# bcaitech1/p4-fr-sorry-math-but-love-you

Hardware: NVIDIA B200
Metric: EfficientSATRN greedy-decode images/sec (higher is better)
Workload: dtype bf16

## Files before the change

### p4-fr-sorry-math-but-love-you_b200/csrc/common.cuh

```cuda
#pragma once
#include <cuda_runtime.h>
#include <cuda_bf16.h>
#include <cuda_fp16.h>
#include <stdint.h>

#if defined(__CUDA_ARCH__) && (__CUDA_ARCH__ < 1000)
#error "frx is written for sm_100a (B200) only"
#endif

namespace frx {

enum Act : int { ACT_NONE = 0, ACT_RELU = 1, ACT_SILU = 2, ACT_SIGMOID = 3, ACT_GELU = 4 };

__device__ __forceinline__ float act_apply(float v, int act) {
  switch (act) {
    case ACT_RELU: return fmaxf(v, 0.f);
    case ACT_SILU: return v / (1.f + expf(-v));
    case ACT_SIGMOID: return 1.f / (1.f + expf(-v));
    case ACT_GELU: return 0.5f * v * (1.f + erff(v * 0.70710678118654752440f));
    default: return v;
  }
}

struct SmemOptIn {
  size_t bytes[64] = {};
  template <class Kernel>
  cudaError_t ensure(Kernel kernel, size_t smem, bool always = false) {
    int dev = 0;
    cudaGetDevice(&dev);
    dev &= 63;
    if ((!always && smem <= 48 * 1024) || (bytes[dev] != 0 && smem <= bytes[dev])) return cudaSuccess;
    cudaError_t e = cudaFuncSetAttribute(kernel, cudaFuncAttributeMaxDynamicSharedMemorySize, (int)smem);
    if (e == cudaSuccess) bytes[dev] = smem;
    return e;
  }
};

#ifndef FRX_ENC_FP16
#define FRX_ENC_FP16 1
#endif
#if FRX_ENC_FP16
typedef __half eh_t;
typedef __half2 eh2_t;
#define FRX_EH_PTX "f16"
__device__ __forceinline__ uint32_t eh2_pack(float lo, float hi) {
  uint32_t r;
  asm("cvt.rn.satfinite.f16x2.f32 %0, %1, %2;\n" : "=r"(r) : "f"(hi), "f"(lo));
  return r;
}
__device__ __forceinline__ eh_t eh_from_float(float f) {
  const uint32_t r = eh2_pack(f, 0.f);
// ... 176 lines not shown
```

### p4-fr-sorry-math-but-love-you_b200/csrc/kernels_bf16.cu

```cuda
#include <cuda_fp16.h>

#include "common.cuh"
#include "kernels.h"

#ifndef FRX_DW_ACC32
#define FRX_DW_ACC32 2
#endif

namespace frx {

namespace {
__device__ __forceinline__ void unpack8(const uint4& u, float (&f)[8]) {
  const uint32_t w[4] = {u.x, u.y, u.z, u.w};
#pragma unroll
  for (int i = 0; i < 4; ++i) {
    const float2 t = eh2_unpack(w[i]);
    f[2 * i] = t.x;
    f[2 * i + 1] = t.y;
  }
}
__device__ __forceinline__ uint4 pack8(const float (&f)[8]) {
  uint32_t w[4];
#pragma unroll
  for (int i = 0; i < 4; ++i) w[i] = eh2_pack(f[2 * i], f[2 * i + 1]);
  return make_uint4(w[0], w[1], w[2], w[3]);
}
}

__global__ void __launch_bounds__(256) stem_conv_bf16_kernel(const float* __restrict__ in, const float* __restrict__ w,
                                                             const float* __restrict__ scale, const float* __restrict__ shift,
                                                             eh_t* __restrict__ out, int B, int Cin, int H, int W,
                                                             int OH, int OW, int Cout) {
  extern __shared__ float ws[];
  for (int i = threadIdx.x; i < Cout * Cin * 9; i += blockDim.x) ws[i] = w[i];
  float* ssc = ws + Cout * Cin * 9;
  float* ssh = ssc + Cout;
  for (int i = threadIdx.x; i < Cout; i += blockDim.x) { ssc[i] = scale[i]; ssh[i] = shift[i]; }
  __syncthreads();
  const int C8 = Cout / 8;
  long long total = (long long)B * OH * OW * C8;
  long long idx = (long long)blockIdx.x * blockDim.x + threadIdx.x;
  if (idx >= total) return;
  const int co0 = (int)(idx % C8) * 8;
  long long pix = idx / C8;
  const int ow = (int)(pix % OW), oh = (int)((pix / OW) % OH), n = (int)(pix / ((long long)OW * OH));
  float acc[8];
#pragma unroll
  for (int j = 0; j < 8; ++j) acc[j] = 0.f;
  for (int ci = 0; ci < Cin; ++ci) {
    const float* ip = in + (((long long)n * Cin + ci) * H + oh * 2) * W + ow * 2;
    float x[9];
#pragma unroll
// ... 16 lines not shown
template <int COUT>
__global__ void __launch_bounds__(128) stem_conv_px_bf16_kernel(const float* __restrict__ in, const float* __restrict__ w,
                                                                const float* __restrict__ scale, const float* __restrict__ shift,
                                                                eh_t* __restrict__ out, int B, int Cin, int H, int W,
                                                                int OH, int OW) {
  extern __shared__ __align__(16) float ws[];
  const int taps = Cin * 9;
  for (int i = threadIdx.x; i < COUT * taps; i += blockDim.x) {
    const int co = i / taps, r = i - co * taps;
    ws[r * COUT + co] = w[i];
  }
  float* ssc = ws + COUT * taps;
  float* ssh = ssc + COUT;
  uint4* stage = reinterpret_cast<uint4*>(ws + ((COUT * taps + 2 * COUT + 3) & ~3));
  for (int i = threadIdx.x; i < COUT; i += blockDim.x) { ssc[i] = scale[i]; ssh[i] = shift[i]; }
  __syncthreads();
  const long long npix = (long long)B * OH * OW, pix0 = (long long)blockIdx.x * blockDim.x;
  const long long pix = min(pix0 + threadIdx.x, npix - 1);
  const int ow = (int)(pix % OW), oh = (int)((pix / OW) % OH), n = (int)(pix / ((long long)OW * OH));
  float acc[COUT];
#pragma unroll
  for (int j = 0; j < COUT; ++j) acc[j] = 0.f;
  for (int ci = 0; ci < Cin; ++ci) {
    const float* ip = in + (((long long)n * Cin + ci) * H + oh * 2) * W + ow * 2;
    float x[9];
#pragma unroll
    for (int kh = 0; kh < 3; ++kh)
#pragma unroll
      for (int kw = 0; kw < 3; ++kw) x[kh * 3 + kw] = __ldg(ip + kh * W + kw);
#pragma unroll
// ... 27 lines not shown
  if (Cout == 24) {
    const long long pixels = (long long)B * OH * OW;
    const int smem24 = ((24 * Cin * 9 + 2 * 24 + 3) & ~3) * sizeof(float) + 128 * 3 * 16;
    stem_conv_px_bf16_kernel<24><<<(unsigned)((pixels + 127) / 128), 128, smem24, st>>>(in, w, scale, shift, out, B, Cin, H, W, OH, OW);
    return;
  }
  long long total = (long long)B * OH * OW * (Cout / 8);
  int smem = (Cout * Cin * 9 + 2 * Cout) * sizeof(float);
  stem_conv_bf16_kernel<<<(unsigned)((total + 255) / 256), 256, smem, st>>>(in, w, scale, shift, out, B, Cin, H, W, OH, OW, Cout);
}

__global__ void __launch_bounds__(256) dwconv3x3_bf16_kernel(const eh_t* __restrict__ in, const float* __restrict__ w,
                                                             const float* __restrict__ scale, const float* __restrict__ shift,
                                                             eh_t* __restrict__ out, int B, int H, int W, int C, int OH,
                                                             int OW, int stride, int pad_t, int pad_l, int act) {
  const int C8 = C >> 3;
  long long total = (long long)B * OH * OW * C8;
  long long idx = (long long)blockIdx.x * blockDim.x + threadIdx.x;
  if (idx >= total) return;
  const int c = (int)(idx % C8) * 8;
  long long pix = idx / C8;
  const int ow = (int)(pix % OW), oh = (int)((pix / OW) % OH), n = (int)(pix / ((long long)OW * OH));
  float acc[8];
#pragma unroll
  for (int j = 0; j < 8; ++j) acc[j] = 0.f;
#pragma unroll
  for (int kh = 0; kh < 3; ++kh) {
    const int ih = oh * stride - pad_t + kh;
    if (ih < 0 || ih >= H) continue;
#pragma unroll
// ... 82 lines not shown

__global__ void __launch_bounds__(256) dwconv_se_mean_kernel(const eh_t* __restrict__ in, const float* __restrict__ w,
                                                             const float* __restrict__ scale, const float* __restrict__ shift,
                                                             eh_t* __restrict__ out, float* __restrict__ mean,
                                                             int H, int W, int C, int OH, int OW, int stride, int pad_t,
                                                             int pad_l, const float* __restrict__ se_w1,
                                                             const float* __restrict__ se_w2, int se_floats) {
  extern __shared__ __align__(16) unsigned char dw_smem[];
  {
    const long long line = ((long long)(blockIdx.y * gridDim.x + blockIdx.x) * blockDim.x + threadIdx.x) * 32;
    if (line < se_floats) {
      asm volatile("prefetch.global.L2 [%0];\n" ::"l"(se_w1 + line));
      asm volatile("prefetch.global.L2 [%0];\n" ::"l"(se_w2 + line));
    }
  }
  uint4* tile = reinterpret_cast<uint4*>(dw_smem);
  float (*red)[64 + 1] = reinterpret_cast<float (*)[64 + 1]>(dw_smem + (size_t)H * W * 8 * 16);
  float* wsm = reinterpret_cast<float*>(dw_smem + (size_t)H * W * 8 * 16 + 32 * 65 * sizeof(float));
  const int n = blockIdx.x, c0 = blockIdx.y * 64;
  const int cg = threadIdx.x & 7, pl = threadIdx.x >> 3;
  const int c = c0 + cg * 8;
  const bool c_ok = c < C;
  const eh_t* ip = in + (long long)n * H * W * C;
  for (int i = threadIdx.x; i < H * W * 8; i += 256) {
    const int px = i >> 3, g = i & 7;
    tile[i] = (c0 + g * 8 < C) ? __ldg(reinterpret_cast<const uint4*>(ip + (long long)px * C + c0 + g * 8)) : make_uint4(0u, 0u, 0u, 0u);
  }
  float sum[8];
#pragma unroll
  for (int j = 0; j < 8; ++j) sum[j] = 0.f;
// ... 62 lines not shown
__global__ void __launch_bounds__(CH * 4) dwconv4_se_mean_kernel(const eh_t* __restrict__ in, const float* __restrict__ w,
                                                                 const float* __restrict__ scale, const float* __restrict__ shift,
                                                                 eh_t* __restrict__ out, float* __restrict__ mean,
                                                                 int H, int W, int C, int OH, int OW, int stride, int pad_t,
                                                                 int pad_l, const float* __restrict__ se_w1,
                                                                 const float* __restrict__ se_w2, int se_floats) {
  constexpr int NT = CH * 4, G8 = CH / 8, G4 = CH / 4;
  extern __shared__ __align__(16) unsigned char dw_smem[];
  {
    const long long line = ((long long)(blockIdx.y * gridDim.x + blockIdx.x) * NT + threadIdx.x) * 32;
    if (line < se_floats) {
      asm volatile("prefetch.global.L2 [%0];\n" ::"l"(se_w1 + line));
      asm volatile("prefetch.global.L2 [%0];\n" ::"l"(se_w2 + line));
    }
  }
  uint4* tile = reinterpret_cast<uint4*>(dw_smem);
  float (*red)[CH + 1] = reinterpret_cast<float (*)[CH + 1]>(dw_smem + (size_t)H * W * G8 * 16);
  const int n = blockIdx.x, c0 = blockIdx.y * CH;
  const eh_t* ip = in + (long long)n * H * W * C;
  for (int i = threadIdx.x; i < H * W * G8; i += NT) {
    const int px = i / G8, g = i - px * G8;
    uint4 v = make_uint4(0u, 0u, 0u, 0u);
    if (c0 + g * 8 < C) {
#if FRX_ENC_FP16
      v = __ldg(reinterpret_cast<const uint4*>(ip + (long long)px * C + c0 + g * 8));
#else
      float x[8];
      unpack8(__ldg(reinterpret_cast<const uint4*>(ip + (long long)px * C + c0 + g * 8)), x);
      const __half2 h0 = __floats2half2_rn(x[0], x[1]), h1 = __floats2half2_rn(x[2], x[3]);
      const __half2 h2 = __floats2half2_rn(x[4], x[5]), h3 = __floats2half2_rn(x[6], x[7]);
// ... 120 lines not shown
    for (int i = 0; i < 16; ++i) s2 += red[i][threadIdx.x];
    mean[(long long)n * C + c0 + threadIdx.x] = s2 / (float)(OH * OW);
  }
}

constexpr int SE_IMGS = 4;
constexpr int SE_ROWS = 4;
__global__ void __launch_bounds__(512, 1) se_fc_kernel(const float* __restrict__ mean, const float* __restrict__ w1,
                                                       const float* __restrict__ b1, const float* __restrict__ w2,
                                                       const float* __restrict__ b2, float* __restrict__ gate, int B, int C,
                                                       int R) {
  extern __shared__ float sm[];
  float* mv = sm;
  float* red = sm + SE_IMGS * C;
  const int n0 = blockIdx.x * SE_IMGS;
  for (int i = threadIdx.x; i < SE_IMGS * C; i += blockDim.x) {
    const int im = i / C;
    mv[i] = n0 + im < B ? mean[(long long)n0 * C + i] : 0.f;
  }
  __syncthreads();
  const int warp = threadIdx.x >> 5, lane = threadIdx.x & 31;
  const int nwarps = blockDim.x >> 5;
  for (int r0 = warp * SE_ROWS; r0 < R; r0 += nwarps * SE_ROWS) {
    float s[SE_ROWS][SE_IMGS];
#pragma unroll
    for (int j = 0; j < SE_ROWS; ++j)
#pragma unroll
      for (int im = 0; im < SE_IMGS; ++im) s[j][im] = 0.f;
#pragma unroll 3
    for (int c4 = lane; c4 < C / 4; c4 += 32) {
// ... 25 lines not shown
    for (int im = 0; im < SE_IMGS; ++im) s[im] = bb;
#pragma unroll 32
    for (int r = 0; r < R; ++r) {
      const float wv = __ldg(w2 + (long long)r * C + c);
#pragma unroll
      for (int im = 0; im < SE_IMGS; ++im) s[im] = fmaf(wv, red[im * R + r], s[im]);
    }
#pragma unroll
    for (int im = 0; im < SE_IMGS; ++im)
      if (n0 + im < B) gate[(long long)(n0 + im) * C + c] = 1.f / (1.f + expf(-s[im]));
  }
}

__global__ void __launch_bounds__(256) se_apply_kernel(eh_t* __restrict__ x, const float* __restrict__ gate,
                                                       long long total8, int HW, int C) {
  long long i = (long long)blockIdx.x * blockDim.x + threadIdx.x;
  if (i >= total8) return;
  const int C8 = C >> 3;
  const int c = (int)(i % C8) * 8;
  const long long n = i / ((long long)C8 * HW);
  uint4* ptr = reinterpret_cast<uint4*>(x) + i;
  float v[8];
  unpack8(*ptr, v);
  const float4 g0 = __ldg(reinterpret_cast<const float4*>(gate + n * C + c));
  const float4 g1 = __ldg(reinterpret_cast<const float4*>(gate + n * C + c + 4));
  v[0] *= g0.x; v[1] *= g0.y; v[2] *= g0.z; v[3] *= g0.w;
  v[4] *= g1.x; v[5] *= g1.y; v[6] *= g1.z; v[7] *= g1.w;
  *ptr = pack8(v);
}

// ... 22 lines not shown

__device__ __forceinline__ uint32_t pack2(float lo, float hi) {
  return eh2_pack(lo, hi);
}
__device__ __forceinline__ void mma16816(float (&c)[4], const uint32_t (&a)[4], uint32_t b0, uint32_t b1) {
  asm("mma.sync.aligned.m16n8k16.row.col.f32." FRX_EH_PTX "." FRX_EH_PTX ".f32 {%0,%1,%2,%3}, {%4,%5,%6,%7}, {%8,%9}, {%0,%1,%2,%3};\n"
      : "+f"(c[0]), "+f"(c[1]), "+f"(c[2]), "+f"(c[3])
      : "r"(a[0]), "r"(a[1]), "r"(a[2]), "r"(a[3]), "r"(b0), "r"(b1));
}

template <int S>
__global__ void __launch_bounds__(S * 2) enc_attn_mma_kernel(const float* __restrict__ qkv,
                                                             eh_t* __restrict__ out,
                                                             int D, int heads, float inv_temp) {
  constexpr int HD = 64, NT = S / 8;
  const int b = blockIdx.x / heads, hh = blockIdx.x % heads;
  const int warp = threadIdx.x >> 5, lane = threadIdx.x & 31, gid = lane >> 2, tig = lane & 3;
  const int ld = 3 * D;
  const float* qb = qkv + (long long)b * S * ld + hh * HD;
  const int i0 = warp * 16;
  float sacc[NT][4];
#pragma unroll
  for (int nt = 0; nt < NT; ++nt)
#pragma unroll
    for (int e = 0; e < 4; ++e) sacc[nt][e] = 0.f;
#pragma unroll
  for (int ks = 0; ks < 4; ++ks) {
    const float* q0 = qb + (long long)(i0 + gid) * ld + 16 * ks + 2 * tig;
    const float* q1 = q0 + 8 * ld;
    const float2 a00 = __ldg(reinterpret_cast<const float2*>(q0)), a10 = __ldg(reinterpret_cast<const float2*>(q1));
// ... 62 lines not shown
  return true;
}

constexpr int C24 = 24, C24_TH = 8, C24_TW = 32, C24_KS = 14;

__global__ void __launch_bounds__(256) conv3x3_c24_mma_kernel(const eh_t* __restrict__ in, const uint2* __restrict__ wfrag,
                                                              const float* __restrict__ scale, const float* __restrict__ shift,
                                                              eh_t* __restrict__ out, int H, int W, int add_res) {
  constexpr int PW = C24_TW + 2, PH = C24_TH + 2;
  __shared__ __align__(16) eh_t halo[PH * PW * C24];
  __shared__ uint2 wsm[C24_KS * 3 * 32];
  const int tiles_x = (W + C24_TW - 1) / C24_TW, tiles_y = (H + C24_TH - 1) / C24_TH;
  const int n = blockIdx.x / (tiles_x * tiles_y), t = blockIdx.x % (tiles_x * tiles_y);
  const int y0 = (t / tiles_x) * C24_TH, x0 = (t % tiles_x) * C24_TW;
  const eh_t* ip = in + (long long)n * H * W * C24;
  for (int i = threadIdx.x; i < PH * PW * 3; i += 256) {
    const int pix = i / 3, ch = i - pix * 3;
    const int py = pix / PW, px = pix - py * PW;
    const int y = y0 + py - 1, x = x0 + px - 1;
    uint4 v = make_uint4(0u, 0u, 0u, 0u);
    if (y >= 0 && y < H && x >= 0 && x < W) v = __ldg(reinterpret_cast<const uint4*>(ip + ((long long)y * W + x) * C24) + ch);
    reinterpret_cast<uint4*>(halo)[i] = v;
  }
  for (int i = threadIdx.x; i < C24_KS * 3 * 32; i += 256) wsm[i] = __ldg(wfrag + i);
  __syncthreads();
  const int warp = threadIdx.x >> 5, lane = threadIdx.x & 31, gid = lane >> 2, tig = lane & 3;
  float acc[2][3][4];
#pragma unroll
  for (int mt = 0; mt < 2; ++mt)
#pragma unroll
    for (int nt = 0; nt < 3; ++nt)
#pragma unroll
      for (int e = 0; e < 4; ++e) acc[mt][nt][e] = 0.f;
  const uint32_t* hw = reinterpret_cast<const uint32_t*>(halo);
#pragma unroll
  for (int s = 0; s < C24_KS; ++s) {
    const int klo = 16 * s, khi = 16 * s + 8;
    const int tap_lo = klo / C24, ch_lo = klo % C24, tap_hi = khi / C24, ch_hi = khi % C24;
    uint32_t a[2][4];
// ... 220 lines not shown
```

### p4-fr-sorry-math-but-love-you_b200/csrc/kernels_f32.cu

```cuda
#include "common.cuh"
#include "kernels.h"

namespace frx {

__global__ void __launch_bounds__(256) stem_conv_kernel(const float* __restrict__ in,
                                                        const float* __restrict__ w,
                                                        const float* __restrict__ scale,
                                                        const float* __restrict__ shift,
                                                        float* __restrict__ out, int B, int Cin, int H,
                                                        int W, int OH, int OW, int Cout, int stride, int pad,
                                                        int act) {
  extern __shared__ float ws[];
  for (int i = threadIdx.x; i < Cout * Cin * 9; i += blockDim.x) ws[i] = w[i];
  float* ssc = ws + Cout * Cin * 9;
  float* ssh = ssc + Cout;
  for (int i = threadIdx.x; i < Cout; i += blockDim.x) { ssc[i] = scale[i]; ssh[i] = shift[i]; }
  __syncthreads();
  long long total = (long long)B * OH * OW * Cout;
  long long idx = (long long)blockIdx.x * blockDim.x + threadIdx.x;
  if (idx >= total) return;
  int co = (int)(idx % Cout);
  long long pix = idx / Cout;
  int ow = (int)(pix % OW);
  int oh = (int)((pix / OW) % OH);
// ... 352 lines not shown
}

void launch_maxpool2_f32(const float* in, float* out, int B, int H, int W, int C, cudaStream_t st) {
  long long total = (long long)B * (H / 2) * (W / 2) * (C / 4);
  maxpool2_f32_kernel<<<(unsigned)((total + 255) / 256), 256, 0, st>>>(in, out, B, H, W, C);
}

__global__ void __launch_bounds__(1024) pe2d_f32_kernel(const float* __restrict__ x,
                                                       const float* __restrict__ w0,
                                                       const float* __restrict__ b0,
                                                       const float* __restrict__ w1,
                                                       const float* __restrict__ b1,
                                                       const float* __restrict__ peh,
                                                       const float* __restrict__ pew,
                                                       float* __restrict__ out, int h, int w, int C) {
  extern __shared__ float sm[];
  float* mean = sm;
  float* hid = sm + C;
  float* g = hid + C / 2;
  const int S = h * w, n = blockIdx.x;
  const float* xp = x + (long long)n * S * C;
  const float inv = 1.f / (float)S;
  for (int c = threadIdx.x; c < C; c += blockDim.x) {
    float s = 0.f;
    for (int q = 0; q < S; ++q) s += __ldg(xp + (long long)q * C + c);
    mean[c] = s * inv;
  }
  __syncthreads();
  const int warp = threadIdx.x >> 5, lane = threadIdx.x & 31;
  const int nwarps = blockDim.x >> 5;
// ... 25 lines not shown
                     cudaStream_t st) {
  int smem = (C + C / 2 + 2 * C) * sizeof(float);
  pe2d_f32_kernel<<<B, 1024, smem, st>>>(x, w0, b0, w1, b1, peh, pew, out, h, w, C);
}

__device__ __forceinline__ void store_as(float* p, float v) { *p = v; }
__device__ __forceinline__ void store_as(eh_t* p, float v) { *p = eh_from_float(v); }

template <typename OutT>
__global__ void __launch_bounds__(256) layernorm_f32_generic_kernel(const float* __restrict__ x,
                                                            const float* __restrict__ res,
                                                            const float* __restrict__ gamma,
                                                            const float* __restrict__ beta,
                                                            OutT* __restrict__ out, int M, int C,
                                                            int scramble_S) {
  const int warp = threadIdx.x >> 5, lane = threadIdx.x & 31;
  const int m = blockIdx.x * 8 + warp;
  if (m >= M) return;
  const float* xp = x + (long long)m * C;
  const float* rp = res ? res + (long long)m * C : nullptr;
  float v[64];
  const int per = C / 32;
  float s = 0.f;
#pragma unroll
  for (int i = 0; i < 64; ++i) {
    if (i < per) {
      float t = __ldg(xp + i * 32 + lane);
      if (rp) t += __ldg(rp + i * 32 + lane);
      v[i] = t;
      s += t;
// ... 17 lines not shown
        store_as(out + ((long long)b * scramble_S + pp) * C + cc, o);
      } else {
        store_as(out + (long long)m * C + ch, o);
      }
    }
  }
}

template <typename OutT, int PER>
__global__ void __launch_bounds__(256) layernorm_f32_kernel(const float* __restrict__ x,
                                                            const float* __restrict__ res,
                                                            const float* __restrict__ gamma,
                                                            const float* __restrict__ beta,
                                                            OutT* __restrict__ out, int M, int C,
                                                            int scramble_S) {
  const int warp = threadIdx.x >> 5, lane = threadIdx.x & 31;
  const int m = blockIdx.x * 8 + warp;
  if (m >= M) return;
  const float* xp = x + (long long)m * C;
  const float* rp = res ? res + (long long)m * C : nullptr;
  float v[PER];
  float s = 0.f;
#pragma unroll
  for (int i = 0; i < PER; ++i) {
    float t = __ldg(xp + i * 32 + lane);
    if (rp) t += __ldg(rp + i * 32 + lane);
    v[i] = t;
    s += t;
  }
  const float mean = warp_sum(s) / (float)C;
// ... 30 lines not shown
  else if (per == 16) layernorm_f32_kernel<OutT, 16><<<g, 256, 0, st>>>(x, res, gamma, beta, out, M, C, scramble_S);
  else if (per == 32) layernorm_f32_kernel<OutT, 32><<<g, 256, 0, st>>>(x, res, gamma, beta, out, M, C, scramble_S);
  else if (per == 64) layernorm_f32_kernel<OutT, 64><<<g, 256, 0, st>>>(x, res, gamma, beta, out, M, C, scramble_S);
  else layernorm_f32_generic_kernel<OutT><<<g, 256, 0, st>>>(x, res, gamma, beta, out, M, C, scramble_S);
}

void launch_layernorm_f32(const float* x, const float* res, const float* gamma, const float* beta,
                          float* out, int M, int C, int scramble_S, cudaStream_t st) {
  layernorm_launch<float>(x, res, gamma, beta, out, M, C, scramble_S, st);
}

__global__ void __launch_bounds__(256) layernorm_scramble_bf16_kernel(const float* __restrict__ x, const float* __restrict__ res,
                                                                      const float* __restrict__ gamma,
                                                                      const float* __restrict__ beta,
                                                                      eh_t* __restrict__ out, int S, int C) {
  extern __shared__ eh_t ln_tile[];
  const int b = blockIdx.x, warp = threadIdx.x >> 5, lane = threadIdx.x & 31;
  const int per = C / 32, LD = S + 2;
  for (int qd = warp; qd < S; qd += 8) {
    const float* xp = x + ((long long)b * S + qd) * C;
    const float* rp = res ? res + ((long long)b * S + qd) * C : nullptr;
    float v[16];
    float s = 0.f;
#pragma unroll
    for (int i = 0; i < 16; ++i)
      if (i < per) {
        float t = __ldg(xp + i * 32 + lane);
        if (rp) t += __ldg(rp + i * 32 + lane);
        v[i] = t;
        s += t;
// ... 25 lines not shown
  const size_t scr_smem = (size_t)C * (scramble_S + 2) * 2;
  static SmemOptIn scr_opt;
  if (scramble_S > 0 && C <= 512 && C % 32 == 0 && M % scramble_S == 0 && scr_smem <= 160 * 1024 &&
      scr_opt.ensure(layernorm_scramble_bf16_kernel, scr_smem) == cudaSuccess) {
    layernorm_scramble_bf16_kernel<<<M / scramble_S, 256, scr_smem, st>>>(x, res, gamma, beta, out,
                                                                                               scramble_S, C);
    return;
  }
  layernorm_launch<eh_t>(x, res, gamma, beta, out, M, C, scramble_S, st);
}

template <typename OutT>
__global__ void __launch_bounds__(128) enc_attn_f32_kernel(const float* __restrict__ qkv,
                                                           OutT* __restrict__ out,
                                                           int S, int D, int heads, float temperature) {
  extern __shared__ float sm[];
  const int HD = D / heads;
  const int LDS_ = HD + 1;
  float* Q = sm;
  float* K = Q + S * LDS_;
  float* V = K + S * LDS_;
  float* P = V + S * LDS_;
  const int b = blockIdx.x / heads, hh = blockIdx.x % heads;
  const float* base = qkv + (long long)b * S * 3 * D + hh * HD;
  for (int i = threadIdx.x; i < S * HD; i += blockDim.x) {
    int r = i / HD, c = i % HD;
    const float* rp = base + (long long)r * 3 * D + c;
    Q[r * LDS_ + c] = __ldg(rp);
    K[r * LDS_ + c] = __ldg(rp + D);
    V[r * LDS_ + c] = __ldg(rp + 2 * D);
// ... 378 lines not shown
```

### p4-fr-sorry-math-but-love-you_b200/csrc/kernels_tc.cu

```cuda
#include <cuda.h>
#include <cuda_fp16.h>
#include <cudaTypedefs.h>

#include <cstdio>
#include <cstdlib>

#include "common.cuh"
#include "kernels.h"

namespace frx {

namespace {

constexpr int TC_BM = 128;
constexpr int TC_BK = 64;
constexpr int TC_STAGES = 3;
constexpr int TC_A_BYTES = TC_BM * TC_BK * 2;

__device__ __forceinline__ uint32_t smem_u32(const void* p) { return (uint32_t)__cvta_generic_to_shared(p); }

__device__ __forceinline__ void cp_async16(uint32_t dst, const void* src, uint32_t src_bytes) {
  asm volatile("cp.async.cg.shared.global [%0], [%1], 16, %2;\n" ::"r"(dst), "l"(src), "r"(src_bytes) : "memory");
}
__device__ __forceinline__ void cp_async_commit() { asm volatile("cp.async.commit_group;\n" ::: "memory"); }
// ... 243 lines not shown

  if (warp == 0) {
    asm volatile("tcgen05.alloc.cta_group::1.sync.aligned.shared::cta.b32 [%0], %1;\n" ::"r"(smem_u32(&tmem_base_s)), "n"(NCOLS) : "memory");
    asm volatile("tcgen05.relinquish_alloc_permit.cta_group::1.sync.aligned;\n" ::: "memory");
  }
  if (tid == 32) {
#pragma unroll
    for (int s = 0; s < TC_STAGES; ++s) mbar_init(&mma_done[s], 1);
    mbar_init(&acc_done, 1);
    asm volatile("fence.mbarrier_init.release.cluster;\n" ::: "memory");
  }
  tc_fence_before();
  __syncthreads();
  tc_fence_after();
  const uint32_t tmem = tmem_base_s;

  const int c = tid & 7, rbase = tid >> 3;
  const eh_t* a_ptr[4];
  int a_ih0[4], a_iw0[4];
  bool a_ok[4];
#pragma unroll
  for (int i = 0; i < 4; ++i) {
    const int m = m0 + rbase + 32 * i;
    a_ok[i] = m < p.M;
    a_ih0[i] = a_iw0[i] = 0;
    a_ptr[i] = p.A;
    if (a_ok[i]) {
      if (p.conv) {
        const int ow = m % p.OW;
        const int t = m / p.OW;
// ... 128 lines not shown
  const int tiles_m = (p.M + TC_BM - 1) / TC_BM;
  const int num_tiles = tiles_m * tiles_n;
  const bool gather = p.conv && !p.im2col;

  if (warp == WS_MMA_WARP) {
    asm volatile("tcgen05.alloc.cta_group::1.sync.aligned.shared::cta.b32 [%0], %1;\n" ::"r"(smem_u32(&tmem_base_s)), "n"(NCOLS) : "memory");
    asm volatile("tcgen05.relinquish_alloc_permit.cta_group::1.sync.aligned;\n" ::: "memory");
  }
  if (tid == 0) {
#pragma unroll
    for (int s = 0; s < WS_STAGES; ++s) { mbar_init(&full_bar[s], (gather ? WS_PROD_THREADS : 0) + 1); mbar_init(&empty_bar[s], 1); }
    mbar_init(&acc_full[0], 1); mbar_init(&acc_full[1], 1);
    const int epi_threads = (WS_EPI_WARPS + (gather ? 0 : WS_PROD_WARPS)) * 32;
    mbar_init(&acc_empty[0], epi_threads); mbar_init(&acc_empty[1], epi_threads);
    asm volatile("fence.mbarrier_init.release.cluster;\n" ::: "memory");
  }
  tc_fence_before();
  __syncthreads();
  tc_fence_after();
  const uint32_t tmem = tmem_base_s;

  if (gather ? warp < WS_PROD_WARPS : warp == WS_TMA_WARP) {
    const bool tma_thread = gather ? tid == 0 : lane == 0;
    const uint32_t tma_bytes = (uint32_t)BN * (TC_BK * 2) + (gather ? 0u : (uint32_t)TC_A_BYTES);
    if (!gather && !tma_thread) {
    } else {
    const int c = tid & 7, rbase = tid >> 3;
    int it = 0;
    for (int tile = blockIdx.x; tile < num_tiles; tile += gridDim.x) {
      const int m0 = (tile / tiles_n) * TC_BM, n0 = (tile % tiles_n) * BN;
      const eh_t* a_ptr[WS_A_PASSES];
      int a_ih0[WS_A_PASSES], a_iw0[WS_A_PASSES];
      bool a_ok[WS_A_PASSES];
      int bw = 0, bh = 0, bn = 0;
      if (p.im2col) {
// ... 300 lines not shown
```

### p4-fr-sorry-math-but-love-you_b200/csrc/runtime.cu

```cuda
#include <cmath>
#include <cstdarg>
#include <cstdio>
#include <cstring>
#include <map>
#include <string>
#include <vector>

#include "../../include/frx.h"
#include "kernels.h"
#include "runtime.h"

using namespace frx;

static int fail(frx_handle* h, const char* fmt, ...) {
  char buf[1024];
  va_list ap;
  va_start(ap, fmt);
  vsnprintf(buf, sizeof buf, fmt, ap);
  va_end(ap);
  if (h) h->err = buf;
  return 1;
}

#define CK(expr)                                                                          \
// ... 26 lines not shown
  ~DeviceGuard() {
    if (changed) cudaSetDevice(prev);
  }
};
#define ON_DEVICE(dev) \
  DeviceGuard guard__;  \
  CK(guard__.enter(dev))

static int dev_alloc(frx_handle* h, void** p, size_t bytes) {
  if (bytes == 0) bytes = 256;
  cudaError_t e = cudaMalloc(p, bytes);
  if (e != cudaSuccess) return fail(h, "cudaMalloc(%zu) failed: %s", bytes, cudaGetErrorString(e));
  h->allocs.push_back(*p);
  h->device_bytes += (int64_t)bytes;
  return 0;
}

struct ArenaBuilder {
  std::vector<float> host;
  size_t add(const float* src, size_t n) {
    size_t off = (host.size() + 63) / 64 * 64;
    host.resize(off + n);
    if (src) memcpy(host.data() + off, src, n * sizeof(float));
    return off;
  }
  float* at(size_t off) { return host.data() + off; }
};

static const HostTensor* find(frx_handle* h, const std::string& name) {
  auto it = h->raw.find(name);
// ... 97 lines not shown
  if (cfg->network == FRX_NET_SWIN && (cfg->height != 384 || cfg->width != 384 || cfg->in_ch != 3 || cfg->enc_hidden != 1024))
    return fail(h, "SWIN is fixed to Swin-B/384: 384x384x3 input, 1024-wide memory (networks/SWIN.py:1028-1031)");
  if (cfg->dec_hidden % cfg->dec_heads || (cfg->dec_hidden / cfg->dec_heads != 32 && cfg->dec_hidden / cfg->dec_heads != 64))
    return fail(h, "decoder head_dim must be 32 or 64");
  if (cfg->dec_hidden > 512) return fail(h, "decoder hidden_dim > 512 not supported");
  if (cfg->max_batch <= 0 || cfg->max_steps <= 0) return fail(h, "max_batch/max_steps must be positive");
  return 0;
}

extern "C" void frx_destroy(frx_handle* h) {
  if (!h) return;
  DeviceGuard guard;
  guard.enter(h->cfg.device);
  frx_train_destroy(h);
  for (auto& kv : h->graphs) cudaGraphExecDestroy(kv.second.exec);
  for (void* p : h->allocs) cudaFree(p);
  for (auto& kv : h->taps) cudaFree(kv.second.data);
  if (h->ev[0]) for (int i = 0; i < 5; ++i) cudaEventDestroy(h->ev[i]);
  for (auto& sl : h->pipe) {
    if (sl.h2d) { cudaEventDestroy(sl.h2d); cudaEventDestroy(sl.enc); cudaEventDestroy(sl.done); cudaEventDestroy(sl.d2h); }
  }
  if (h->pipe_h2d) { cudaStreamDestroy(h->pipe_h2d); cudaStreamDestroy(h->pipe_d2h); cudaStreamDestroy(h->pipe_enc); }
  delete h;
}

extern "C" int frx_load_tensor(frx_handle* h, const char* name, const void* data, const int64_t* shape,
                               int32_t ndim, int32_t dtype) {
  if (!h || !name || !data) return fail(h, "frx_load_tensor: null argument");
  HostTensor t;
  size_t n = 1;
// ... 6 lines not shown
    CK(cudaMemcpy(tmp.data(), data, n * sizeof(int64_t), cudaMemcpyDefault));
    t.f.resize(n);
    for (size_t i = 0; i < n; ++i) t.f[i] = (float)tmp[i];
  } else {
    return fail(h, "frx_load_tensor('%s'): unsupported dtype %d", name, dtype);
  }
  h->raw[name] = std::move(t);
  h->finalized = false;
  return 0;
}

extern "C" int frx_set_option(frx_handle* h, const char* key, int64_t value) {
  if (!h || !key) return 1;
  ON_DEVICE(h->cfg.device);
  std::string k(key);
  if (k == "taps") h->opt_taps = value != 0;
  else if (k == "graphs") h->opt_graphs = value != 0;
  else if (k == "step16") h->opt_step16 = value != 0;
  else if (k == "pipe_enc") h->opt_pipe_enc = value != 0;
  else if (k == "timing") h->opt_timing = value != 0;
  else if (k == "cluster_images") {}
  else if (k == "dec_hpc") h->opt_dec_hpc = (value == 1 || value == 2) ? (int)value : 0;
  else if (k == "conv24") h->opt_conv24 = value != 0;
  else if (k == "enc_fp32") h->opt_enc_fp32 = value != 0;
  else if (k == "tc_ws") h->opt_tc_ws = value != 0;
  else if (k == "train_splitk") h->opt_train_splitk = value != 0;
  else if (k == "tc_im2col") h->opt_tc_im2col = value != 0;
  else if (k == "prof") {
    h->opt_prof = value != 0;
    if (h->opt_prof && !h->prof) { void* p; if (dev_alloc(h, &p, 16 * 8)) return 1; h->prof = (long long*)p; }
  }
  else if (k == "parts") {
    if (h->ws_ready && ((int)value & 3) != h->opt_parts)
      return fail(h, "option 'parts' cannot change after the first frx_finalize_weights (create a new handle)");
    h->opt_parts = (int)value & 3;
    h->finalized = false;
  }
  else return fail(h, "unknown option '%s'", key);
  return 0;
// ... 584 lines not shown
    if (c.precision == FRX_PREC_BF16) {
      if (dev_alloc(h, &p, L * B * T * D * 2)) return 1; h->kself_bf = p;
      if (dev_alloc(h, &p, L * B * T * D * 2)) return 1; h->vself_bf = p;
      if (dev_alloc(h, &p, L * B * S * D * 2)) return 1; h->kcross_bf = p;
      if (dev_alloc(h, &p, L * B * S * D * 2)) return 1; h->vcross_bf = p;
      if (dev_alloc(h, &p, B * S * (size_t)c.dec_src * 2)) return 1; h->mem_bf = p;
    }
    }
    if (dev_alloc(h, &p, B * S * C * 4)) return 1; h->memory_int = (float*)p;
    if (dev_alloc(h, &p, (size_t)c.in_ch * c.height * c.width * B * 4)) return 1; h->images_int = (float*)p;
    for (int i = 0; i < 5; ++i) CK(cudaEventCreate(&h->ev[i]));
    h->ws_ready = true;
  }
  for (auto& kv : h->graphs) cudaGraphExecDestroy(kv.second.exec);
  h->graphs.clear();
  h->finalized = true;
  return 0;
}

static int tap(frx_handle* h, const std::string& name, const float* src, int B, int H, int W, int C,
               cudaStream_t st) {
  if (!h->opt_taps) return 0;
  Tap& t = h->taps[name];
  size_t n = (size_t)B * H * W * C;
  if (t.capacity < n) {
    if (t.data) cudaFree(t.data);
    CK(cudaMalloc((void**)&t.data, n * 4));
    t.capacity = n;
  }
  t.shape[0] = B; t.shape[1] = H; t.shape[2] = W; t.shape[3] = C;
// ... 223 lines not shown
  const int fh = h->feat_h, fw = h->feat_w, S = fh * fw, C = c.enc_hidden, F = c.enc_filter, M = B * S;
  float* tf = (float*)y;
  {
    TcGemmP g = tc_dense(x, M, 256, A, h->last_wb, C, tf, 1);
    g.scale = A + h->last_sc; g.shift = A + h->last_sh; g.act = ACT_SILU;
    TCL(g);
  }
  if (tap(h, "trunk", tf, B, fh, fw, C, st)) return 1;
  float* xf = (float*)x;
  launch_pe2d_f32(tf, A + h->pe_w0, A + h->pe_b0, A + h->pe_w1, A + h->pe_b1, A + h->pe_h, A + h->pe_w, xf, B, fh, fw, C, st);
  CKL();
  if (tap(h, "pe2d", xf, B, fh, fw, C, st)) return 1;
  return encoder_layers_16(h, tf, xf, m0, m1, B, memory, st);
}

static int encode_swin(frx_handle* h, const float* images, int B, float* memory, cudaStream_t st) {
  const float* A = h->arena;
  float* x = h->sw_x[0];
  float* y = h->sw_x[1];
  launch_swin_patch_embed(images, A + h->sw_pe_w, A + h->sw_pe_b, A + h->sw_pe_g, A + h->sw_pe_beta, A + h->sw_ape, x, B, 384,
                          96, 128, st);
  CKL();
  if (tap(h, "embed", x, B, 96, 96, 128, st)) return 1;
  size_t bi = 0;
  const int depths[4] = {2, 2, 18, 2};
  for (int i = 0; i < 4; ++i) {
    for (int j = 0; j < depths[i]; ++j, ++bi) {
      const SwinBlockW& b = h->sw_blocks[bi];
      const int M = B * b.res * b.res, C = b.dim;
      if (h->cfg.precision == FRX_PREC_BF16) {
// ... 98 lines not shown
  if (H != h->feat_h || W != h->feat_w) return fail(h, "trunk output %dx%d != expected %dx%d", H, W, h->feat_h, h->feat_w);
  *out = y;
  return 0;
}

extern "C" int frx_encode(frx_handle* h, const float* images, int32_t B, float* memory, void* stream) {
  if (!h) return 1;
  if (!h->finalized) return fail(h, "frx_encode: weights not finalized");
  if (!(h->opt_parts & 1)) return fail(h, "frx_encode: handle was created without the encoder part");
  if (B <= 0 || B > h->cfg.max_batch) return fail(h, "frx_encode: batch %d outside (0, %d]", B, h->cfg.max_batch);
  const frx_config& c = h->cfg;
  cudaStream_t st = (cudaStream_t)stream;
  ON_DEVICE(c.device);
  if (c.network == FRX_NET_SWIN) return encode_swin(h, images, B, memory, st);
  if (c.precision == FRX_PREC_BF16 && !h->opt_enc_fp32 && c.network == FRX_NET_EFFICIENT_SATRN)
    return encode_bf16(h, images, B, memory, st);
  const float* A = h->arena;
  float* t = nullptr;
  if (c.network == FRX_NET_LITE_SATRN) {
    if (run_trunk_lite(h, images, B, &t, st)) return 1;
  } else if (run_trunk_efficientnet(h, images, B, &t, st)) {
    return 1;
  }
  const int fh = h->feat_h, fw = h->feat_w, S = fh * fw, C = c.enc_hidden, F = c.enc_filter;
  if (tap(h, "trunk", t, B, fh, fw, C, st)) return 1;
  float* x = (t == h->act[0]) ? h->act[1] : h->act[0];
  launch_pe2d_f32(t, A + h->pe_w0, A + h->pe_b0, A + h->pe_w1, A + h->pe_b1, A + h->pe_h, A + h->pe_w, x, B, fh, fw, C, st);
  CKL();
  if (tap(h, "pe2d", x, B, fh, fw, C, st)) return 1;
  if (c.network == FRX_NET_LITE_SATRN && c.precision == FRX_PREC_BF16 && !h->opt_enc_fp32 && h->enc[0].wb_qkv)
    return encoder_layers_16(h, t, x, (eh_t*)h->mid[0], (eh_t*)h->mid[1], B, memory, st);
// ... 692 lines not shown
```

### p4-fr-sorry-math-but-love-you_b200/csrc/runtime.h

```cpp
#pragma once
#include <cuda_runtime.h>
#include <stdint.h>

#include <map>
#include <string>
#include <tuple>
#include <vector>

#include "../../include/frx.h"

struct HostTensor {
  std::vector<int64_t> shape;
  std::vector<float> f;
};

struct BlockW {
  int kind;
  int cin, cout, k, stride, mid, se_r;
  bool residual;
  std::string name;
  size_t w_a, sc_a, sh_a;
  size_t w_dw, sc_dw, sh_dw;
  size_t se_w1, se_b1, se_w2, se_b2, se_w2t = 0;
  size_t w_b, sc_b, sh_b;
// ... 13 lines not shown
  size_t wb_o = 0, wb_q2 = 0, wb_o2 = 0, wb_f0 = 0, wb_f1 = 0, wb_sqkv = 0;
  size_t ln1_g, ln1_b, ln2_g, ln2_b, ln3_g, ln3_b;
};
struct FusedW { size_t wt, b; int N; };
struct SwinBlockW {
  int dim, res, heads, ws, shift;
  size_t n1_g, n1_b, bias_table, qkv_w, qkv_b, proj_w, proj_b, n2_g, n2_b, fc1_w, fc1_b, fc2_w, fc2_b;
  size_t qkv_wb = 0, proj_wb = 0, fc1_wb = 0, fc2_wb = 0;
};
struct SwinMergeW { int dim, res; size_t red_w, n_g, n_b; size_t red_wb = 0; };
struct DecPackW { size_t w_o, w_q2, w_o2, w_f0, w_f1, w_next; };
struct Tap { float* data = nullptr; size_t capacity = 0; int shape[4] = {0, 0, 0, 0}; };
typedef std::tuple<int, int, int> GraphKey;
struct GraphEntry { cudaGraphExec_t exec; int64_t nodes; int64_t last_use = 0; };
constexpr size_t FRX_MAX_GRAPHS = 4;

struct BeamWs {
  double *hscore = nullptr, *nlogp = nullptr;
  int *hnode = nullptr, *nprev = nullptr, *ntok = nullptr, *nlen = nullptr, *nkv = nullptr, *chain = nullptr, *small = nullptr;
  float* logits = nullptr;
  int* host_flag = nullptr;
};
struct TfWs {
  float *x = nullptr, *y = nullptr, *z = nullptr, *qkv = nullptr, *ff = nullptr;
  unsigned char* mask = nullptr;
  void *xb = nullptr, *ffb = nullptr;
};

struct frx_handle {
  frx_config cfg{};
  std::string err;
  int num_sms = 0;
  std::map<std::string, HostTensor> raw;
  bool finalized = false, ws_ready = false;
  bool opt_taps = false, opt_graphs = true, opt_timing = false, opt_step16 = true, opt_pipe_enc = true;
  int* step_hist = nullptr;
  bool opt_prof = false;
  bool opt_tc_im2col = true;
  void* hook_wpad = nullptr; size_t hook_wpad_bytes = 0;
  bool opt_tc_ws = true;
  int opt_dec_hpc = 0;
  bool opt_conv24 = true;
  bool opt_enc_fp32 = false;
  long long* prof = nullptr;
  int opt_parts = 3;
  int feat_h = 0, feat_w = 0;
  std::vector<void*> allocs;
  int64_t device_bytes = 0, launches = 0;

  float* arena = nullptr;
  size_t arena_bytes = 0;
  size_t stem_w = 0, stem_sc = 0, stem_sh = 0, last_w = 0, last_sc = 0, last_sh = 0;
  std::vector<BlockW> blocks;
  LiteConvW lite[4]{};
  size_t pe_w0 = 0, pe_b0 = 0, pe_w1 = 0, pe_b1 = 0, pe_h = 0, pe_w = 0;
  std::vector<EncLayerW> enc;
  size_t sw_pe_w = 0, sw_pe_b = 0, sw_pe_g = 0, sw_pe_beta = 0, sw_ape = 0, sw_norm_g = 0, sw_norm_b = 0;
  std::vector<SwinBlockW> sw_blocks;
// ... 8 lines not shown
  size_t dpack_first = 0;
  std::vector<DecPackW> dpack2;
  size_t dpack2_first = 0;

  float *act[2] = {nullptr, nullptr}, *mid[2] = {nullptr, nullptr}, *gate = nullptr;
  float *kself = nullptr, *vself = nullptr, *cross = nullptr;
  float *dx = nullptr, *dqkv = nullptr, *datt = nullptr, *dpre1 = nullptr, *dpre2 = nullptr, *du = nullptr,
        *dw = nullptr, *dq2 = nullptr, *dff = nullptr;
  float *logits_int = nullptr, *memory_int = nullptr, *images_int = nullptr;
  long long *tokens_int = nullptr, *forced_int = nullptr;
  int* cur_tok = nullptr;
  void* mem_bf = nullptr;
  void *kself_bf = nullptr, *vself_bf = nullptr, *kcross_bf = nullptr, *vcross_bf = nullptr;

  std::map<GraphKey, GraphEntry> graphs;
  int64_t graph_clock = 0;
  std::map<std::string, Tap> taps;
  cudaEvent_t ev[5] = {nullptr, nullptr, nullptr, nullptr, nullptr};
  struct PipeSlot {
    float *img = nullptr, *mem = nullptr;
    long long* tok = nullptr;
    cudaEvent_t h2d = nullptr, enc = nullptr, done = nullptr, d2h = nullptr;
    bool busy = false;
  };
  PipeSlot pipe[2];
  cudaStream_t pipe_h2d = nullptr, pipe_d2h = nullptr, pipe_enc = nullptr;
  float last_ms[4] = {0, 0, 0, 0};
  BeamWs beam;
  TfWs tf;
  int step_idx = 0, step_batch = 0;
// ... 11 lines not shown
```

Before: 12960.

## Capture bf16 encoder into a CUDA graph with programmatic dependent launch edges

Captures the bf16 EfficientSATRN encoder into a cached CUDA graph, keyed by batch size and buffer pointers, on the second call with the same key. Kernel-to-kernel edges are rewritten as programmatic dependencies, and griddepcontrol wait/trigger calls are added to the encoder kernels so each kernel's prologue (weight loads, barrier and TMEM setup, tensormap prefetch) can overlap the tail of the previous one. This is meant to cut per-launch host overhead and inter-kernel gaps. It risks correctness problems if any kernel reads predecessor data before its wait, and graphs are dropped on any option change.

```diff
diff --git a/p4-fr-sorry-math-but-love-you_b200/csrc/common.cuh b/p4-fr-sorry-math-but-love-you_b200/csrc/common.cuh
--- a/p4-fr-sorry-math-but-love-you_b200/csrc/common.cuh
+++ b/p4-fr-sorry-math-but-love-you_b200/csrc/common.cuh
@@ -35,6 +35,9 @@
     return e;
   }
 };
+
+__device__ __forceinline__ void pdl_wait() { asm volatile("griddepcontrol.wait;\n" ::: "memory"); }
+__device__ __forceinline__ void pdl_trigger() { asm volatile("griddepcontrol.launch_dependents;\n" ::: "memory"); }
 
 #ifndef FRX_ENC_FP16
 #define FRX_ENC_FP16 1
diff --git a/p4-fr-sorry-math-but-love-you_b200/csrc/kernels_bf16.cu b/p4-fr-sorry-math-but-love-you_b200/csrc/kernels_bf16.cu
--- a/p4-fr-sorry-math-but-love-you_b200/csrc/kernels_bf16.cu
+++ b/p4-fr-sorry-math-but-love-you_b200/csrc/kernels_bf16.cu
@@ -36,6 +36,8 @@
   float* ssc = ws + Cout * Cin * 9;
   float* ssh = ssc + Cout;
   for (int i = threadIdx.x; i < Cout; i += blockDim.x) { ssc[i] = scale[i]; ssh[i] = shift[i]; }
+  pdl_wait();
+  pdl_trigger();
   __syncthreads();
   const int C8 = Cout / 8;
   long long total = (long long)B * OH * OW * C8;
@@ -82,6 +84,8 @@
   float* ssh = ssc + COUT;
   uint4* stage = reinterpret_cast<uint4*>(ws + ((COUT * taps + 2 * COUT + 3) & ~3));
   for (int i = threadIdx.x; i < COUT; i += blockDim.x) { ssc[i] = scale[i]; ssh[i] = shift[i]; }
+  pdl_wait();
+  pdl_trigger();
   __syncthreads();
   const long long npix = (long long)B * OH * OW, pix0 = (long long)blockIdx.x * blockDim.x;
   const long long pix = min(pix0 + threadIdx.x, npix - 1);
@@ -139,6 +143,8 @@
                                                              const float* __restrict__ scale, const float* __restrict__ shift,
                                                              eh_t* __restrict__ out, int B, int H, int W, int C, int OH,
                                                              int OW, int stride, int pad_t, int pad_l, int act) {
+  pdl_wait();
+  pdl_trigger();
   const int C8 = C >> 3;
   long long total = (long long)B * OH * OW * C8;
   long long idx = (long long)blockIdx.x * blockDim.x + threadIdx.x;
@@ -251,6 +257,8 @@
       asm volatile("prefetch.global.L2 [%0];\n" ::"l"(se_w2 + line));
     }
   }
+  pdl_wait();
+  pdl_trigger();
   uint4* tile = reinterpret_cast<uint4*>(dw_smem);
   float (*red)[64 + 1] = reinterpret_cast<float (*)[64 + 1]>(dw_smem + (size_t)H * W * 8 * 16);
   float* wsm = reinterpret_cast<float*>(dw_smem + (size_t)H * W * 8 * 16 + 32 * 65 * sizeof(float));
@@ -343,6 +351,8 @@
       asm volatile("prefetch.global.L2 [%0];\n" ::"l"(se_w2 + line));
     }
   }
+  pdl_wait();
+  pdl_trigger();
   uint4* tile = reinterpret_cast<uint4*>(dw_smem);
   float (*red)[CH + 1] = reinterpret_cast<float (*)[CH + 1]>(dw_smem + (size_t)H * W * G8 * 16);
   const int n = blockIdx.x, c0 = blockIdx.y * CH;
@@ -493,6 +503,8 @@
   float* mv = sm;
   float* red = sm + SE_IMGS * C;
   const int n0 = blockIdx.x * SE_IMGS;
+  pdl_wait();
+  pdl_trigger();
   for (int i = threadIdx.x; i < SE_IMGS * C; i += blockDim.x) {
     const int im = i / C;
     mv[i] = n0 + im < B ? mean[(long long)n0 * C + i] : 0.f;
@@ -548,6 +560,8 @@
 
 __global__ void __launch_bounds__(256) se_apply_kernel(eh_t* __restrict__ x, const float* __restrict__ gate,
                                                        long long total8, int HW, int C) {
+  pdl_wait();
+  pdl_trigger();
   long long i = (long long)blockIdx.x * blockDim.x + threadIdx.x;
   if (i >= total8) return;
   const int C8 = C >> 3;
@@ -600,6 +614,8 @@
                                                              eh_t* __restrict__ out,
                                                              int D, int heads, float inv_temp) {
   constexpr int HD = 64, NT = S / 8;
+  pdl_wait();
+  pdl_trigger();
   const int b = blockIdx.x / heads, hh = blockIdx.x % heads;
   const int warp = threadIdx.x >> 5, lane = threadIdx.x & 31, gid = lane >> 2, tig = lane & 3;
   const int ld = 3 * D;
@@ -692,6 +708,9 @@
   const int n = blockIdx.x / (tiles_x * tiles_y), t = blockIdx.x % (tiles_x * tiles_y);
   const int y0 = (t / tiles_x) * C24_TH, x0 = (t % tiles_x) * C24_TW;
   const eh_t* ip = in + (long long)n * H * W * C24;
+  for (int i = threadIdx.x; i < C24_KS * 3 * 32; i += 256) wsm[i] = __ldg(wfrag + i);
+  pdl_wait();
+  pdl_trigger();
   for (int i = threadIdx.x; i < PH * PW * 3; i += 256) {
     const int pix = i / 3, ch = i - pix * 3;
     const int py = pix / PW, px = pix - py * PW;
@@ -700,7 +719,6 @@
     if (y >= 0 && y < H && x >= 0 && x < W) v = __ldg(reinterpret_cast<const uint4*>(ip + ((long long)y * W + x) * C24) + ch);
     reinterpret_cast<uint4*>(halo)[i] = v;
   }
-  for (int i = threadIdx.x; i < C24_KS * 3 * 32; i += 256) wsm[i] = __ldg(wfrag + i);
   __syncthreads();
   const int warp = threadIdx.x >> 5, lane = threadIdx.x & 31, gid = lane >> 2, tig = lane & 3;
   float acc[2][3][4];
diff --git a/p4-fr-sorry-math-but-love-you_b200/csrc/kernels_f32.cu b/p4-fr-sorry-math-but-love-you_b200/csrc/kernels_f32.cu
--- a/p4-fr-sorry-math-but-love-you_b200/csrc/kernels_f32.cu
+++ b/p4-fr-sorry-math-but-love-you_b200/csrc/kernels_f32.cu
@@ -390,6 +390,8 @@
                                                        const float* __restrict__ peh,
                                                        const float* __restrict__ pew,
                                                        float* __restrict__ out, int h, int w, int C) {
+  pdl_wait();
+  pdl_trigger();
   extern __shared__ float sm[];
   float* mean = sm;
   float* hid = sm + C;
@@ -445,6 +447,8 @@
                                                             const float* __restrict__ beta,
                                                             OutT* __restrict__ out, int M, int C,
                                                             int scramble_S) {
+  pdl_wait();
+  pdl_trigger();
   const int warp = threadIdx.x >> 5, lane = threadIdx.x & 31;
   const int m = blockIdx.x * 8 + warp;
   if (m >= M) return;
@@ -492,6 +496,8 @@
                                                             const float* __restrict__ beta,
                                                             OutT* __restrict__ out, int M, int C,
                                                             int scramble_S) {
+  pdl_wait();
+  pdl_trigger();
   const int warp = threadIdx.x >> 5, lane = threadIdx.x & 31;
   const int m = blockIdx.x * 8 + warp;
   if (m >= M) return;
@@ -552,6 +558,8 @@
                                                                       const float* __restrict__ gamma,
                                                                       const float* __restrict__ beta,
                                                                       eh_t* __restrict__ out, int S, int C) {
+  pdl_wait();
+  pdl_trigger();
   extern __shared__ eh_t ln_tile[];
   const int b = blockIdx.x, warp = threadIdx.x >> 5, lane = threadIdx.x & 31;
   const int per = C / 32, LD = S + 2;
@@ -607,6 +615,8 @@
 __global__ void __launch_bounds__(128) enc_attn_f32_kernel(const float* __restrict__ qkv,
                                                            OutT* __restrict__ out,
                                                            int S, int D, int heads, float temperature) {
+  pdl_wait();
+  pdl_trigger();
   extern __shared__ float sm[];
   const int HD = D / heads;
   const int LDS_ = HD + 1;
diff --git a/p4-fr-sorry-math-but-love-you_b200/csrc/kernels_tc.cu b/p4-fr-sorry-math-but-love-you_b200/csrc/kernels_tc.cu
--- a/p4-fr-sorry-math-but-love-you_b200/csrc/kernels_tc.cu
+++ b/p4-fr-sorry-math-but-love-you_b200/csrc/kernels_tc.cu
@@ -281,6 +281,8 @@
   __syncthreads();
   tc_fence_after();
   const uint32_t tmem = tmem_base_s;
+  pdl_wait();
+  pdl_trigger();
 
   const int c = tid & 7, rbase = tid >> 3;
   const eh_t* a_ptr[4];
@@ -439,11 +441,15 @@
     const int epi_threads = (WS_EPI_WARPS + (gather ? 0 : WS_PROD_WARPS)) * 32;
     mbar_init(&acc_empty[0], epi_threads); mbar_init(&acc_empty[1], epi_threads);
     asm volatile("fence.mbarrier_init.release.cluster;\n" ::: "memory");
+    asm volatile("prefetch.tensormap [%0];\n" ::"l"(reinterpret_cast<uint64_t>(&tmA)) : "memory");
+    asm volatile("prefetch.tensormap [%0];\n" ::"l"(reinterpret_cast<uint64_t>(&tmW)) : "memory");
   }
   tc_fence_before();
   __syncthreads();
   tc_fence_after();
   const uint32_t tmem = tmem_base_s;
+  pdl_wait();
+  pdl_trigger();
 
   if (gather ? warp < WS_PROD_WARPS : warp == WS_TMA_WARP) {
     const bool tma_thread = gather ? tid == 0 : lane == 0;
diff --git a/p4-fr-sorry-math-but-love-you_b200/csrc/runtime.cu b/p4-fr-sorry-math-but-love-you_b200/csrc/runtime.cu
--- a/p4-fr-sorry-math-but-love-you_b200/csrc/runtime.cu
+++ b/p4-fr-sorry-math-but-love-you_b200/csrc/runtime.cu
@@ -64,6 +64,12 @@
   h->allocs.push_back(*p);
   h->device_bytes += (int64_t)bytes;
   return 0;
+}
+
+static void drop_enc_graphs(frx_handle* h) {
+  for (auto& kv : h->enc_graphs)
+    if (kv.second.exec) cudaGraphExecDestroy(kv.second.exec);
+  h->enc_graphs.clear();
 }
 
 struct ArenaBuilder {
@@ -191,6 +197,7 @@
   guard.enter(h->cfg.device);
   frx_train_destroy(h);
   for (auto& kv : h->graphs) cudaGraphExecDestroy(kv.second.exec);
+  drop_enc_graphs(h);
   for (void* p : h->allocs) cudaFree(p);
   for (auto& kv : h->taps) cudaFree(kv.second.data);
   if (h->ev[0]) for (int i = 0; i < 5; ++i) cudaEventDestroy(h->ev[i]);
@@ -227,6 +234,7 @@
   if (!h || !key) return 1;
   ON_DEVICE(h->cfg.device);
   std::string k(key);
+  drop_enc_graphs(h);
   if (k == "taps") h->opt_taps = value != 0;
   else if (k == "graphs") h->opt_graphs = value != 0;
   else if (k == "step16") h->opt_step16 = value != 0;
@@ -236,6 +244,7 @@
   else if (k == "dec_hpc") h->opt_dec_hpc = (value == 1 || value == 2) ? (int)value : 0;
   else if (k == "conv24") h->opt_conv24 = value != 0;
   else if (k == "enc_fp32") h->opt_enc_fp32 = value != 0;
+  else if (k == "enc_graph") h->opt_enc_graph = value != 0;
   else if (k == "tc_ws") h->opt_tc_ws = value != 0;
   else if (k == "train_splitk") h->opt_train_splitk = value != 0;
   else if (k == "tc_im2col") h->opt_tc_im2col = value != 0;
@@ -850,6 +859,7 @@
   }
   for (auto& kv : h->graphs) cudaGraphExecDestroy(kv.second.exec);
   h->graphs.clear();
+  drop_enc_graphs(h);
   h->finalized = true;
   return 0;
 }
@@ -1103,6 +1113,71 @@
   return encoder_layers_16(h, tf, xf, m0, m1, B, memory, st);
 }
 
+static cudaError_t make_edges_programmatic(cudaGraph_t g) {
+  size_t n = 0;
+  cudaError_t e = cudaGraphGetEdges_v2(g, nullptr, nullptr, nullptr, &n);
+  if (e != cudaSuccess || n == 0) return e;
+  std::vector<cudaGraphNode_t> from(n), to(n);
+  std::vector<cudaGraphEdgeData> data(n);
+  e = cudaGraphGetEdges_v2(g, from.data(), to.data(), data.data(), &n);
+  cudaGraphEdgeData pdl{};
+  pdl.from_port = cudaGraphKernelNodePortProgrammatic;
+  pdl.type = cudaGraphDependencyTypeProgrammatic;
+  for (size_t i = 0; i < n && e == cudaSuccess; ++i) {
+    cudaGraphNodeType tf, tt;
+    if ((e = cudaGraphNodeGetType(from[i], &tf)) != cudaSuccess || (e = cudaGraphNodeGetType(to[i], &tt)) != cudaSuccess) break;
+    if (tf != cudaGraphNodeTypeKernel || tt != cudaGraphNodeTypeKernel || data[i].type != cudaGraphDependencyTypeDefault) continue;
+    e = cudaGraphRemoveDependencies_v2(g, &from[i], &to[i], &data[i], 1);
+    if (e == cudaSuccess) e = cudaGraphAddDependencies_v2(g, &from[i], &to[i], &pdl, 1);
+  }
+  return e;
+}
+
+static int encode_bf16_graph(frx_handle* h, const float* images, int B, float* memory, cudaStream_t st) {
+  const EncGraphKey key{B, images, memory};
+  auto it = h->enc_graphs.find(key);
+  const bool first = it == h->enc_graphs.end();
+  if (first) {
+    if (h->enc_graphs.size() >= FRX_MAX_ENC_GRAPHS) {
+      auto victim = h->enc_graphs.begin();
+      for (auto g = h->enc_graphs.begin(); g != h->enc_graphs.end(); ++g)
+        if (g->second.last_use < victim->second.last_use) victim = g;
+      if (victim->second.exec) cudaGraphExecDestroy(victim->second.exec);
+      h->enc_graphs.erase(victim);
+    }
+    it = h->enc_graphs.emplace(key, GraphEntry{nullptr, 0}).first;
+  }
+  GraphEntry& ge = it->second;
+  ge.last_use = ++h->graph_clock;
+  if (ge.exec) {
+    CK(cudaGraphLaunch(ge.exec, st));
+    h->launches += ge.nodes;
+    return 0;
+  }
+  if (encode_bf16(h, images, B, memory, st)) return 1;
+  if (first) return 0;
+  cudaStream_t cs;
+  CK(cudaStreamCreateWithFlags(&cs, cudaStreamNonBlocking));
+  const int64_t before = h->launches;
+  cudaError_t e = cudaStreamBeginCapture(cs, cudaStreamCaptureModeThreadLocal);
+  if (e != cudaSuccess) { cudaStreamDestroy(cs); return fail(h, "encoder graph capture failed: %s", cudaGetErrorString(e)); }
+  const int rc = encode_bf16(h, images, B, memory, cs);
+  cudaGraph_t graph = nullptr;
+  e = cudaStreamEndCapture(cs, &graph);
+  cudaStreamDestroy(cs);
+  const int64_t nodes = h->launches - before;
+  h->launches = before;
+  if (rc) { if (graph) cudaGraphDestroy(graph); return 1; }
+  if (e == cudaSuccess) e = make_edges_programmatic(graph);
+  cudaGraphExec_t exec = nullptr;
+  if (e == cudaSuccess) e = cudaGraphInstantiate(&exec, graph, 0);
+  if (graph) cudaGraphDestroy(graph);
+  if (e != cudaSuccess) return fail(h, "encoder graph capture failed: %s", cudaGetErrorString(e));
+  ge.exec = exec;
+  ge.nodes = nodes;
+  return 0;
+}
+
 static int encode_swin(frx_handle* h, const float* images, int B, float* memory, cudaStream_t st) {
   const float* A = h->arena;
   float* x = h->sw_x[0];
@@ -1231,7 +1306,8 @@
   ON_DEVICE(c.device);
   if (c.network == FRX_NET_SWIN) return encode_swin(h, images, B, memory, st);
   if (c.precision == FRX_PREC_BF16 && !h->opt_enc_fp32 && c.network == FRX_NET_EFFICIENT_SATRN)
-    return encode_bf16(h, images, B, memory, st);
+    return (h->opt_enc_graph && !h->opt_taps) ? encode_bf16_graph(h, images, B, memory, st)
+                                              : encode_bf16(h, images, B, memory, st);
   const float* A = h->arena;
   float* t = nullptr;
   if (c.network == FRX_NET_LITE_SATRN) {
diff --git a/p4-fr-sorry-math-but-love-you_b200/csrc/runtime.h b/p4-fr-sorry-math-but-love-you_b200/csrc/runtime.h
--- a/p4-fr-sorry-math-but-love-you_b200/csrc/runtime.h
+++ b/p4-fr-sorry-math-but-love-you_b200/csrc/runtime.h
@@ -51,6 +51,8 @@
 typedef std::tuple<int, int, int> GraphKey;
 struct GraphEntry { cudaGraphExec_t exec; int64_t nodes; int64_t last_use = 0; };
 constexpr size_t FRX_MAX_GRAPHS = 4;
+typedef std::tuple<int, const void*, const void*> EncGraphKey;
+constexpr size_t FRX_MAX_ENC_GRAPHS = 8;
 
 struct BeamWs {
   double *hscore = nullptr, *nlogp = nullptr;
@@ -79,6 +81,7 @@
   int opt_dec_hpc = 0;
   bool opt_conv24 = true;
   bool opt_enc_fp32 = false;
+  bool opt_enc_graph = true;
   long long* prof = nullptr;
   int opt_parts = 3;
   int feat_h = 0, feat_w = 0;
@@ -117,6 +120,7 @@
   void *kself_bf = nullptr, *vself_bf = nullptr, *kcross_bf = nullptr, *vcross_bf = nullptr;
 
   std::map<GraphKey, GraphEntry> graphs;
+  std::map<EncGraphKey, GraphEntry> enc_graphs;
   int64_t graph_clock = 0;
   std::map<std::string, Tap> taps;
   cudaEvent_t ev[5] = {nullptr, nullptr, nullptr, nullptr, nullptr};
```

After: 13190, median of 6. 1.02x the previous value.
